# SMART-TTS/SMART-NAR_Fast_TTS

Hardware: AMD Instinct MI355X
Metric: mel_frames_per_sec (higher is better)
Workload: dtype f32

## Files before the change

smart-nar_fast_tts_amd/csrc/gemm_conv.hip:

```cpp
#include <hip/hip_ext.h>
#include <cstdlib>
#include <cstring>
#include <type_traits>
#include "rowln.h"

namespace ns {

typedef float f32x16 __attribute__((ext_vector_type(16)));
typedef unsigned u32x4g __attribute__((ext_vector_type(4)));
typedef __attribute__((address_space(3))) void* lds_ptr_t;

[[maybe_unused]] constexpr int OOR = (int)0x80000000;

template <int BM, int BN, int BK, int KS, int WGM = 2, int WGN = 2, bool ROWEPI = false, int TICKET = 0, int MF = 32>
__global__ __launch_bounds__(64 * WGM * WGN * KS) void k_conv_gemm(ConvGemm p, int ntn, int fl) {
#if defined(__HIP_DEVICE_COMPILE__)
  constexpr int NW = WGM * WGN;
  constexpr int WM = BM / WGM, WN = BN / WGN;
  constexpr int TM = WM / MF, TN = WN / MF;
  constexpr int NR = MF == 32 ? 16 : 4;
  constexpr int LG = 64 / MF;
  constexpr int KG = 4 * LG;
  constexpr int CPR = BK / 4;
  constexpr int RPI = 64 / CPR;
  static_assert(MF == 32 || MF == 16, "MFMA tile edge");
  static_assert(TM >= 1 && TN >= 1 && WM % MF == 0 && WN % MF == 0 && BM % RPI == 0 && BN % RPI == 0 && BK % KG == 0, "tile / wave-grid geometry");
  constexpr int FSH = (BK == 64) ? 0 : (BK == 32) ? 1 : 2;
  constexpr int FMSK = CPR - 1;
  static_assert(BK == 64 || BK == 32 || BK == 16, "BK");
  constexpr int EPR = 2 * BK;
  constexpr int NPASS = (BM + EPR - 1) / EPR;
  static_assert(!ROWEPI || (KS == 1 && BN % 256 == 0 && (BM % EPR) % NW == 0 && (BM < EPR || EPR % NW == 0)), "row epilogue: every pass's rows divide over the waves");
  static_assert(!(ROWEPI && TICKET), "a full-row tile needs no ticket");
  using acc_t = typename std::conditional<MF == 32, f32x16, f32x4>::type;
  constexpr bool ACC2 = TM * TN * NR <= 32;

  __shared__ __attribute__((aligned(16))) float As0[KS * BM * BK];
  __shared__ __attribute__((aligned(16))) float As1[KS * BM * BK];
  __shared__ __attribute__((aligned(16))) float Bs0[KS * BN * BK];
  __shared__ __attribute__((aligned(16))) float Bs1[KS * BN * BK];

  const int nblk = gridDim.x, bid = blockIdx.x;
  const int q8 = nblk >> 3, r8 = nblk & 7, xcd = bid & 7;
  int pos = (xcd < r8 ? xcd * (q8 + 1) : r8 * (q8 + 1) + (xcd - r8) * q8) + (bid >> 3);
  const int ntm = nblk / ntn, mq = ntm >> 3, mr = ntm & 7;
  int tile_m = 0, tile_n = 0, mstart = 0;
  for (int x = 0; x < 8; ++x) {
    const int gm = mq + (x < mr ? 1 : 0), gsz = gm * ntn;
    if (pos < gsz) {
      tile_n = pos / gm;
      tile_m = mstart + pos % gm;
      break;
    }
    pos -= gsz;
    mstart += gm;
  }
  const int m0 = tile_m * BM, n0 = tile_n * BN;

  const int tid = threadIdx.x, lane = tid & 63;
  const int wall = __builtin_amdgcn_readfirstlane(tid >> 6);
  const int grp = wall / NW, wid = wall % NW;
  const int wm0 = (wid / WGN) * WM, wn0 = (wid % WGN) * WN;

  const int Kt = p.ldw ? p.ldw : p.KW * p.Cin;
  const int cpj = p.Cin / BK;
  const int nch = p.KW * cpj;

  const __amdgpu_buffer_rsrc_t rsA = __builtin_amdgcn_make_buffer_rsrc(
      (void*)(p.X + ((ptrdiff_t)m0 - p.pad) * p.ldx), (short)0, 0x7FFFFFFF, 0x00020000);
  const __amdgpu_buffer_rsrc_t rsB =
      __builtin_amdgcn_make_buffer_rsrc((void*)(p.W + (size_t)n0 * Kt), (short)0, 0x7FFFFFFF, 0x00020000);

  constexpr int TOTA = BM / RPI, TOTB = BN / RPI;
  constexpr int IA = (TOTA + NW - 1) / NW, IB = (TOTB + NW - 1) / NW;
  constexpr bool A_EVEN = TOTA % NW == 0, B_EVEN = TOTB % NW == 0;
  const int lr = lane / CPR, ls = lane % CPR;
  auto ea = [&](int i) { return A_EVEN ? wid * IA + i : i * NW + wid; };
  auto eb = [&](int i) { return B_EVEN ? wid * IB + i : i * NW + wid; };
  int a_base[IA];
  unsigned a_jlo[IA], a_jn[IA];
#pragma unroll
  for (int i = 0; i < IA; ++i) {
    const int r = ea(i) * RPI + lr;
    const int m = m0 + r;
    int t = -1, sw = p.S;
    if (m < p.M) {
      const int mg = m + p.m_base;
      if (p.rm.row_t) { t = p.rm.row_t[mg]; sw = p.rm.row_w[mg]; }
      else t = mg % p.S;
    }
    a_base[i] = (r * p.ldx + (ls ^ ((r >> FSH) & FMSK)) * 4) * 4;
    const int jlo = max(0, p.pad - t), jhi = min(p.KW, sw + p.pad - t);
    a_jlo[i] = (unsigned)jlo;
    a_jn[i] = (t >= 0 && jhi > jlo) ? (unsigned)(jhi - jlo) : 0u;
  }
  int vb[IB];
#pragma unroll
  for (int i = 0; i < IB; ++i) {
    const int r = eb(i) * RPI + lr;
    vb[i] = (n0 + r < p.N) ? (r * Kt + (ls ^ ((r >> FSH) & FMSK)) * 4) * 4 : OOR;
  }
  auto dma_chunk = [&](float* As, float* Bs, int ch) {
    const int cc = ch / p.KW, j = ch - cc * p.KW;
    const int soA = (cc * BK + j * p.ldx) * 4, soB = (j * p.Cin + cc * BK) * 4;
#pragma unroll
    for (int i = 0; i < IA; ++i) {
      const int va = ((unsigned)j - a_jlo[i] < a_jn[i]) ? a_base[i] : OOR;
      if (A_EVEN || ea(i) < TOTA)
        __builtin_amdgcn_raw_ptr_buffer_load_lds(rsA, (lds_ptr_t)&As[ea(i) * RPI * BK], 16, va, soA, 0, 0);
    }
#pragma unroll
    for (int i = 0; i < IB; ++i) {
      if (B_EVEN || eb(i) < TOTB)
        __builtin_amdgcn_raw_ptr_buffer_load_lds(rsB, (lds_ptr_t)&Bs[eb(i) * RPI * BK], 16, vb[i], soB, 0, 0);
    }
  };

  acc_t acc[TM][TN];
#pragma unroll
  for (int mi = 0; mi < TM; ++mi)
#pragma unroll
    for (int ni = 0; ni < TN; ++ni)
#pragma unroll
      for (int r = 0; r < NR; ++r) acc[mi][ni][r] = 0.f;
  [[maybe_unused]] acc_t tot[ACC2 ? TM : 1][ACC2 ? TN : 1];
  if constexpr (ACC2) {
#pragma unroll
    for (int mi = 0; mi < TM; ++mi)
#pragma unroll
      for (int ni = 0; ni < TN; ++ni)
#pragma unroll
        for (int r = 0; r < NR; ++r) tot[mi][ni][r] = 0.f;
  }

  [[maybe_unused]] float bvp[TN];
  if constexpr (KS == 1) {
#pragma unroll
    for (int ni = 0; ni < TN; ++ni) {
      const int n = n0 + wn0 + ni * MF + (lane & (MF - 1));
      bvp[ni] = (p.bias && n < p.N) ? p.bias[n] : 0.f;
    }
  }

  const int frow = lane & (MF - 1), fh = lane / MF;
  int foff[BK / KG];
#pragma unroll
  for (int g = 0; g < BK / KG; ++g) foff[g] = frow * BK + (((LG * g + fh) ^ ((frow >> FSH) & FMSK)) * 4);

  float* const A0 = As0 + grp * BM * BK;
  float* const A1 = As1 + grp * BM * BK;
  float* const B0 = Bs0 + grp * BN * BK;
  float* const B1 = Bs1 + grp * BN * BK;

  const int nsteps = (nch + KS - 1) / KS;
  if (grp < nch) dma_chunk(A0, B0, grp);
  __syncthreads();

  auto step = [&](auto fresh_c, int st, const float* Ac, const float* Bc, float* An, float* Bn) {
    constexpr bool FRESH = decltype(fresh_c)::value;
    const acc_t zero = {};
    const int ch = st * KS + grp;
    if (ch + KS < nch) dma_chunk(An, Bn, ch + KS);
    if (KS == 1 || ch < nch) {
      const float* as = Ac + wm0 * BK;
      const float* bs = Bc + wn0 * BK;
#pragma unroll
      for (int g = 0; g < BK / KG; ++g) {
        if constexpr (MF == 32) {
          f32x4 a[TM], b[TN];
#pragma unroll
          for (int mi = 0; mi < TM; ++mi) a[mi] = *reinterpret_cast<const f32x4*>(as + mi * 32 * BK + foff[g]);
#pragma unroll
          for (int ni = 0; ni < TN; ++ni) b[ni] = *reinterpret_cast<const f32x4*>(bs + ni * 32 * BK + foff[g]);
#pragma unroll
          for (int e = 0; e < 4; ++e)
#pragma unroll
            for (int mi = 0; mi < TM; ++mi)
#pragma unroll
              for (int ni = 0; ni < TN; ++ni)
                acc[mi][ni] = __builtin_amdgcn_mfma_f32_32x32x2f32(a[mi][e], b[ni][e], (FRESH && g == 0 && e == 0) ? zero : acc[mi][ni], 0, 0, 0);
        } else {
          f32x4 b[TN];
#pragma unroll
          for (int ni = 0; ni < TN; ++ni) b[ni] = *reinterpret_cast<const f32x4*>(bs + ni * 16 * BK + foff[g]);
#pragma unroll
          for (int mi = 0; mi < TM; ++mi) {
            const f32x4 a = *reinterpret_cast<const f32x4*>(as + mi * 16 * BK + foff[g]);
#pragma unroll
            for (int e = 0; e < 4; ++e)
#pragma unroll
              for (int ni = 0; ni < TN; ++ni)
                acc[mi][ni] = __builtin_amdgcn_mfma_f32_16x16x4f32(a[e], b[ni][e], (FRESH && g == 0 && e == 0) ? zero : acc[mi][ni], 0, 0, 0);
          }
        }
      }
    } else if constexpr (FRESH) {
#pragma unroll
      for (int mi = 0; mi < TM; ++mi)
#pragma unroll
        for (int ni = 0; ni < TN; ++ni) acc[mi][ni] = zero;
    }
    __syncthreads();
  };
  int due = fl;
  bool fresh = false;
  constexpr std::false_type CONT{};
  constexpr std::true_type OPEN{};
  for (int st = 0; st < nsteps; st += 2) {
    if (ACC2 && fresh) step(OPEN, st, A0, B0, A1, B1);
    else step(CONT, st, A0, B0, A1, B1);
    if (st + 1 < nsteps) step(CONT, st + 1, A1, B1, A0, B0);
    if constexpr (ACC2) {
      due -= 2;
      fresh = due == 0 && st + 2 < nsteps;
      if (fresh) {
        due = fl;
#pragma unroll
        for (int mi = 0; mi < TM; ++mi)
#pragma unroll
          for (int ni = 0; ni < TN; ++ni) tot[mi][ni] += acc[mi][ni];
      }
    }
  }
  if constexpr (ACC2) {
#pragma unroll
    for (int mi = 0; mi < TM; ++mi)
#pragma unroll
      for (int ni = 0; ni < TN; ++ni) acc[mi][ni] = tot[mi][ni] + acc[mi][ni];
  }

  const int ecol = lane & (MF - 1);
  auto crow = [&](int r) { return MF == 32 ? (r & 3) + 8 * (r >> 2) + 4 * (lane >> 5) : r + 4 * (lane >> 4); };
  if constexpr (KS > 1) {
    constexpr int RS = BN + 8, TILE = BM * RS;
    constexpr int PB = (KS * BN * BK) / TILE, PA = (KS * BM * BK) / TILE;
    static_assert(2 * PB + 2 * PA >= KS, "the KS partial tiles must fit the four staging objects, whole tiles per object");
    auto part = [&](int g) -> float* {
      if (g < PB) return Bs0 + g * TILE;
      if (g < 2 * PB) return Bs1 + (g - PB) * TILE;
      if (g < 2 * PB + PA) return As0 + (g - 2 * PB) * TILE;
      return As1 + (g - 2 * PB - PA) * TILE;
    };
    constexpr int NT = 64 * NW * KS, U = BM * BN / 4, UPT = (U + NT - 1) / NT, CPRW = BN / 4;
    f32x4 bia[UPT], res[UPT];
#pragma unroll
    for (int k = 0; k < UPT; ++k) {
      const int u = tid + k * NT, row = u / CPRW, m = m0 + row, n = n0 + (u % CPRW) * 4;
      const bool ok = u < U && m < p.M && n < p.N;
      bia[k] = (ok && p.bias) ? *reinterpret_cast<const f32x4*>(p.bias + n) : f32x4{0.f, 0.f, 0.f, 0.f};
      res[k] = (ok && p.resid) ? *reinterpret_cast<const f32x4*>(p.resid + (size_t)m * p.ldr + n) : f32x4{0.f, 0.f, 0.f, 0.f};
    }
    {
      float* mine = part(grp);
#pragma unroll
      for (int mi = 0; mi < TM; ++mi)
#pragma unroll
        for (int ni = 0; ni < TN; ++ni)
#pragma unroll
          for (int r = 0; r < NR; ++r)
            mine[(wm0 + mi * MF + crow(r)) * RS + wn0 + ni * MF + ecol] = acc[mi][ni][r];
    }
    __syncthreads();
    [[maybe_unused]] const __amdgpu_buffer_rsrc_t rsYs = __builtin_amdgcn_make_buffer_rsrc((void*)p.Y, (short)0, 0x7FFFFFFF, 0x00020000);
#pragma unroll
    for (int k = 0; k < UPT; ++k) {
      const int u = tid + k * NT, row = u / CPRW, c4 = u % CPRW, m = m0 + row, n = n0 + c4 * 4;
      if (u >= U || m >= p.M || n >= p.N) continue;
      f32x4 v = *reinterpret_cast<const f32x4*>(part(0) + row * RS + c4 * 4);
#pragma unroll
      for (int g2 = 1; g2 < KS; ++g2) v += *reinterpret_cast<const f32x4*>(part(g2) + row * RS + c4 * 4);
      v += bia[k];
      if (p.act == ACT_RELU) {
#pragma unroll
        for (int e = 0; e < 4; ++e) v[e] = v[e] > 0.f ? v[e] : 0.f;
      } else if (p.act == ACT_TANH) {
#pragma unroll
        for (int e = 0; e < 4; ++e) v[e] = tanhf(v[e]);
      }
      if (p.resid) v += res[k];
      if constexpr (TICKET != 0) __builtin_amdgcn_raw_buffer_store_b128(__builtin_bit_cast(u32x4g, v), rsYs, (m * p.ldy + n) * 4, 0, 16 );
      else *reinterpret_cast<f32x4*>(p.Y + (size_t)m * p.ldy + n) = v;
    }
  }

  if constexpr (ROWEPI) {
    static_assert(WGM == 1, "full-row tiles put their waves side by side");
    auto trow = [&](int ml) -> float* { return (ml < BK ? Bs0 : Bs1) + (ml % BK) * BN; };
    constexpr int NV = BN / 256;
    f32x4 lng[NV], lnb[NV];
#pragma unroll
    for (int i = 0; i < NV; ++i) {
      lng[i] = *reinterpret_cast<const f32x4*>(p.e.ln_g + lane * 4 + i * 256);
      lnb[i] = *reinterpret_cast<const f32x4*>(p.e.ln_b + lane * 4 + i * 256);
    }
    const RowEpilogue& e2 = p.e;
    auto pass = [&](auto pc) {
      constexpr int P = decltype(pc)::value;
      constexpr int P0 = P * EPR, PR = (BM - P0 < EPR ? BM - P0 : EPR), RPW = PR / NW;
      if constexpr (P > 0) __syncthreads();
      const int mw = m0 + P0 + wid * RPW;
      f32x4 rv[RPW][NV];
#pragma unroll
      for (int rr = 0; rr < RPW; ++rr) {
        const int m = mw + rr;
#pragma unroll
        for (int i = 0; i < NV; ++i) {
          rv[rr][i] = f32x4{0.f, 0.f, 0.f, 0.f};
          if (p.resid && m < p.M) rv[rr][i] = *reinterpret_cast<const f32x4*>(p.resid + (size_t)m * p.ldr + lane * 4 + i * 256);
        }
      }
      int tt[RPW];
      unsigned keep[RPW];
      int mv = mw;
      asm("" : "+v"(mv));
      row_batch_masks<RPW>(p.e, p.M, p.S, mv, 1, tt, keep);
#pragma unroll
      for (int ni = 0; ni < TN; ++ni) {
        const int nl = wn0 + ni * MF + ecol;
        const float bv = bvp[ni];
#pragma unroll
        for (int mi = 0; mi < TM; ++mi) {
          if ((mi * MF) / EPR != P) continue;
#pragma unroll
          for (int r = 0; r < NR; ++r) {
            const int ml = mi * MF + crow(r) - P0;
            float v = acc[mi][ni][r] + bv;
            if (p.act == ACT_RELU) v = v > 0.f ? v : 0.f;
            else if (p.act == ACT_TANH) v = tanhf(v);
            trow(ml)[nl] = v;
          }
        }
      }
      __syncthreads();
      f32x4 v[RPW][NV];
#pragma unroll
      for (int rr = 0; rr < RPW; ++rr)
#pragma unroll
        for (int i = 0; i < NV; ++i) {
          v[rr][i] = *reinterpret_cast<const f32x4*>(trow(wid * RPW + rr) + lane * 4 + i * 256);
          if (p.resid) v[rr][i] += rv[rr][i];
        }
      row_batch_finish<NV, RPW>(v, tt, keep, lane, p.epi, e2, p.M, mv, 1, lng, lnb);
    };
    pass(std::integral_constant<int, 0>{});
    if constexpr (NPASS > 1) pass(std::integral_constant<int, 1>{});
    if constexpr (NPASS > 2) pass(std::integral_constant<int, 2>{});
    if constexpr (NPASS > 3) pass(std::integral_constant<int, 3>{});
    static_assert(NPASS <= 4, "row epilogue: at most 4 parking passes (BM <= 8 BK)");
  } else {
    if constexpr (KS == 1) {
#pragma unroll
    for (int ni = 0; ni < TN; ++ni) {
      const int n = n0 + wn0 + ni * MF + ecol;
      if (n >= p.N) continue;
      const float bv = bvp[ni];
#pragma unroll
      for (int mi = 0; mi < TM; ++mi) {
        float rs[NR];
#pragma unroll
        for (int r = 0; r < NR; ++r) {
          const int m = m0 + wm0 + mi * MF + crow(r);
          rs[r] = (p.resid && m < p.M) ? p.resid[(size_t)m * p.ldr + n] : 0.f;
        }
#pragma unroll
        for (int r = 0; r < NR; ++r) {
          const int m = m0 + wm0 + mi * MF + crow(r);
          if (m >= p.M) continue;
          float v = acc[mi][ni][r] + bv;
          if (p.act == ACT_RELU) v = v > 0.f ? v : 0.f;
          else if (p.act == ACT_TANH) v = tanhf(v);
          if (p.resid) v += rs[r];
          if constexpr (TICKET) __hip_atomic_store(p.Y + (size_t)m * p.ldy + n, v, __ATOMIC_RELAXED, __HIP_MEMORY_SCOPE_AGENT);
          else p.Y[(size_t)m * p.ldy + n] = v;
        }
      }
    }
    }
    if constexpr (TICKET) {
      constexpr int NWALL = NW * KS;
      asm volatile("s_waitcnt vmcnt(0)" ::: "memory");
      __syncthreads();
      int* const last = reinterpret_cast<int*>(As0);
      if (tid == 0) *last = __hip_atomic_fetch_add(p.e.ticket + tile_m, 1, __ATOMIC_RELAXED, __HIP_MEMORY_SCOPE_AGENT) == ntn - 1;
      __syncthreads();
      if (!*last) return;
      const __amdgpu_buffer_rsrc_t rsY = __builtin_amdgcn_make_buffer_rsrc((void*)p.Y, (short)0, p.M * p.ldy * 4, 0x00020000);
      constexpr int RPW = BM / NWALL, RB = RPW < 8 ? RPW : 8;
      static_assert(BM % NWALL == 0 && RPW % RB == 0, "rows divide evenly over the waves");
#pragma unroll
      for (int j0 = 0; j0 < RPW; j0 += RB)
        row_epilogue_batch<TICKET, RB>(rsY, p.ldy, lane, p.epi, p.e, p.M, p.S, m0 + wall + j0 * NWALL, NWALL);
    }
  }
#endif
}

int conv_gemm_acc_chunk() {
  static const int v = [] {
    const char* e = getenv("NS_ACC_CHUNK");
    int k = e ? atoi(e) : 64;
    if (k < 0 || k % 64 != 0) k = 64;
    return k;
  }();
  return v;
}
static int acc_chunk_k() { return conv_gemm_acc_chunk(); }
static int long_k_threshold() {
  static const int v = [] { const char* e = getenv("NS_LONG_K"); const int k = e ? atoi(e) : 512; return k >= 256 ? k : 256; }();
  return v;
}
static constexpr bool tile_chunks(int bm, int bn, int waves) { return bm * bn / (64 * waves) <= 32; }

struct LaunchRecord { int n; int out[2][8]; };
static thread_local LaunchRecord* t_describe = nullptr;

template <int BM, int BN, int BK, int KS = 1, int WGM = 2, int WGN = 2, bool ROWEPI = false, int TICKET = 0, int MF = 32>
static hipError_t launch_t(const ConvGemm& p, hipStream_t st, const LaunchTiming* tm = nullptr) {
  if (LaunchRecord* r = t_describe) {
    if (r->n < 2) {
      const int form[8] = {BM, BN, BK, KS, MF, ROWEPI ? 1 : 0, TICKET, p.M};
      for (int i = 0; i < 8; ++i) r->out[r->n][i] = form[i];
    }
    r->n++;
    return hipSuccess;
  }
  const int ntm = (p.M + BM - 1) / BM, ntn = (p.N + BN - 1) / BN;
  const int fl = ((acc_chunk_k() / BK) + 1) & ~1;
  if (tm && (tm->start || tm->stop))
    hipExtLaunchKernelGGL((k_conv_gemm<BM, BN, BK, KS, WGM, WGN, ROWEPI, TICKET, MF>), dim3(ntm * ntn), dim3(64 * WGM * WGN * KS), 0, st, tm->start, tm->stop, 0, p, ntn, fl);
  else
    hipLaunchKernelGGL((k_conv_gemm<BM, BN, BK, KS, WGM, WGN, ROWEPI, TICKET, MF>), dim3(ntm * ntn), dim3(64 * WGM * WGN * KS), 0, st, p, ntn, fl);
  return hipGetLastError();
}

bool conv_gemm_ticket_ok(int M, int N, int Cin) {
  return M > 0 && (N == 256 || N == 512) && Cin % 32 == 0 && (long long)M * N * 4 < (1ll << 31) && (long)((M + 31) / 32) * ((N + 127) / 128) <= 512;
}

bool conv_gemm_row_epilogue_ok(int M, int N, int Cin) {
  return M > 0 && (N == 256 || N == 512) && Cin % 32 == 0;
}

bool launch_planner_enabled() {
  static const bool on = [] { const char* e = getenv("NS_PLAN"); return !(e && e[0] == '0'); }();
  return on;
}

static ConvGemm row_range(const ConvGemm& p, int begin, int count) {
  ConvGemm q = p;
  q.X += (size_t)begin * p.ldx;
  q.Y += (size_t)begin * p.ldy;
  if (q.resid) q.resid += (size_t)begin * p.ldr;
  q.M = count;
  q.m_base = p.m_base + begin;
  return q;
}

struct TileModel { int bm, bn; float a0, a1, b0, b1; };
enum TileId { T256, T128, T64W, T64, T64N, T32, N_TILES };
static constexpr TileModel kTile[N_TILES] = {
    {256, 256, 11.0f, 0.00f, 10.0f, 7.25f},
    {128, 256, 5.0f, 0.20f, 8.0f, 3.60f},
    {64, 256, 6.0f, 0.17f, 3.6f, 1.83f},
    {64, 128, 5.5f, 0.09f, 1.6f, 0.93f},
    {64, 64, 5.0f, 0.20f, 1.2f, 0.46f},
    {32, 128, 5.0f, 0.23f, 1.0f, 0.45f},
};
static long tile_wgs(int t, long M, int N) { return ((M + kTile[t].bm - 1) / kTile[t].bm) * ((N + kTile[t].bn - 1) / kTile[t].bn); }
static float tile_time(int t, long M, int N, int chunks) {
  const long steps = (tile_wgs(t, M, N) + 255) / 256;
  const float a = kTile[t].a0 + kTile[t].a1 * chunks, b = kTile[t].b0 + kTile[t].b1 * chunks;
  const float more = (t == T64N || t == T32) ? 1.15f : 1.0f;
  return (a + b + b * more * (float)(steps - 1)) * (1.0f + 0.01f * (float)t);
}
enum TileFam { F32 = 0, F16W = 1, F16N = 2 };
struct TileSel { int fam, id; };
static int sel_bm(TileSel t) { return t.fam == F32 ? kTile[t.id].bm : 16 * t.id; }
static int sel_bn(TileSel t) { return t.fam == F32 ? kTile[t.id].bn : t.fam == F16W ? 256 : 128; }
constexpr int F16W_MIN = 3, F16W_MAX = 16, F16N_MIN = 3, F16N_MAX = 10;
static bool tile16_enabled() {
  static const bool on = [] { const char* e = getenv("NS_TILE16"); return !(e && e[0] == '0'); }();
  return on;
}
bool conv_gemm_tile16_enabled() { return launch_planner_enabled() && tile16_enabled(); }
static bool tile16n_enabled() {
  static const bool on = [] { const char* e = getenv("NS_TILE16N"); return !(e && e[0] == '0'); }();
  return on;
}
static float tile16_time(int fam, int slabs, long M, int N, int chunks) {
  const int bm = 16 * slabs, bn = fam == F16W ? 256 : 128;
  const long wgs = ((M + bm - 1) / bm) * ((N + bn - 1) / bn);
  const float steps = (float)((wgs + 255) / 256);
  const float rows = (float)bm * (fam == F16W ? 1.0f : 0.5f);
  const float b1 = 0.0281f * rows * (fam == F16N ? 1.02f : 1.0f);
  return 5.0f + 0.0016f * rows * (float)chunks + steps * (8.0f + b1 * (float)chunks);
}
template <int S>
static hipError_t launch_f16w(const ConvGemm& p, hipStream_t st, const LaunchTiming* tm) { return launch_t<16 * S, 256, 32, 1, 1, 16, false, 0, 16>(p, st, tm); }
template <int S>
static hipError_t launch_f16n(const ConvGemm& p, hipStream_t st, const LaunchTiming* tm) { return launch_t<16 * S, 128, 32, 1, 1, 8, false, 0, 16>(p, st, tm); }
static hipError_t launch_tile(TileSel t, const ConvGemm& p, hipStream_t st, const LaunchTiming* tm) {
  if (t.fam == F16W) {
    switch (t.id) {
      case 3: return launch_f16w<3>(p, st, tm); case 4: return launch_f16w<4>(p, st, tm); case 5: return launch_f16w<5>(p, st, tm);
      case 6: return launch_f16w<6>(p, st, tm); case 7: return launch_f16w<7>(p, st, tm); case 8: return launch_f16w<8>(p, st, tm);
      case 9: return launch_f16w<9>(p, st, tm); case 10: return launch_f16w<10>(p, st, tm); case 11: return launch_f16w<11>(p, st, tm);
      case 12: return launch_f16w<12>(p, st, tm); case 13: return launch_f16w<13>(p, st, tm); case 14: return launch_f16w<14>(p, st, tm);
      case 15: return launch_f16w<15>(p, st, tm); case 16: return launch_f16w<16>(p, st, tm);
      default: return hipErrorInvalidValue;
    }
  }
  if (t.fam == F16N) {
    switch (t.id) {
      case 3: return launch_f16n<3>(p, st, tm); case 4: return launch_f16n<4>(p, st, tm); case 5: return launch_f16n<5>(p, st, tm);
      case 6: return launch_f16n<6>(p, st, tm); case 7: return launch_f16n<7>(p, st, tm); case 8: return launch_f16n<8>(p, st, tm);
      case 9: return launch_f16n<9>(p, st, tm); case 10: return launch_f16n<10>(p, st, tm);
      default: return hipErrorInvalidValue;
    }
  }
  switch (t.id) {
    case T256: return launch_t<256, 256, 32, 1, 8, 2>(p, st, tm);
    case T128: return launch_t<128, 256, 32, 1, 4, 4>(p, st, tm);
    case T64W: return launch_t<64, 256, 32, 1, 2, 4>(p, st, tm);
    case T64: return launch_t<64, 128, 32, 1, 2, 4>(p, st, tm);
    case T64N: return launch_t<64, 64, 32, 1, 2, 2>(p, st, tm);
    default: return launch_t<32, 128, 32, 1, 1, 4>(p, st, tm);
  }
}
struct RowPlan { TileSel main; int main_rows; TileSel rem; float us; };
static RowPlan plan_rows(long M, int N, int chunks) {
  constexpr float CUT_US = 3.0f;
  RowPlan best{{F32, -1}, 0, {F32, T64}, 1e30f};
  const bool long_k = chunks * 32 > long_k_threshold() && acc_chunk_k() > 0;
  const int first = chunks <= 16 ? T64W : long_k ? T128 : T256;
  for (int t = first; t < N_TILES; ++t) {
    if (kTile[t].bn > N && t != T32 && t != T64N && t != T64) continue;
    const float c = tile_time(t, M, N, chunks);
    if (c < best.us) best = RowPlan{{F32, -1}, 0, {F32, t}, c};
  }
  for (int t = first; t <= T64; ++t) {
    if (kTile[t].bn > N) continue;
    const long ntn = (N + kTile[t].bn - 1) / kTile[t].bn;
    const long per = (256 / ntn) * kTile[t].bm;
    if (per <= 0) continue;
    for (long k = M / per; k >= 1 && k >= M / per - 1; --k) {
      const long rows = k * per, rest = M - rows;
      if (rest <= 0) continue;
      const float cm = tile_time(t, rows, N, chunks);
      for (int r = t + 1; r < N_TILES; ++r) {
        if (kTile[r].bn > N && r < T64) continue;
        const float c = cm + CUT_US + tile_time(r, rest, N, chunks);
        if (c < best.us) best = RowPlan{{F32, t}, (int)rows, {F32, r}, c};
      }
    }
  }
  if (tile16_enabled()) {
    float margin = 1.01f;
    if (best.main_rows == 0 && best.rem.fam == F32) {
      const long w = tile_wgs(best.rem.id, M, N);
      if ((double)w / (double)(((w + 255) / 256) * 256) >= 0.9) margin = 1.03f;
    }
    const int w_max = long_k ? 8 : F16W_MAX, n_max = long_k ? 8 : F16N_MAX;
    if (N % 256 == 0)
      for (int sl = F16W_MIN; sl <= w_max; ++sl) {
        const float c = tile16_time(F16W, sl, M, N, chunks) * margin;
        if (c < best.us) best = RowPlan{{F32, -1}, 0, {F16W, sl}, c};
      }
    if (N % 128 == 0 && tile16n_enabled())
      for (int sl = F16N_MIN; sl <= n_max; ++sl) {
        const float c = tile16_time(F16N, sl, M, N, chunks) * margin;
        if (c < best.us) best = RowPlan{{F32, -1}, 0, {F16N, sl}, c};
      }
  }
  return best;
}

bool conv_gemm_plan(int M, int N, int Cin, int KW, int out[8]) {
  if (!launch_planner_enabled() || M <= 0 || N < 128 || Cin % 32 != 0) return false;
  const long rows64 = ((long)M + 63) / 64;
  if (rows64 * ((N + 127) / 128) <= 256) return false;
  const RowPlan pl = plan_rows(M, N, KW * (Cin / 32));
  const TileSel mt = pl.main_rows ? pl.main : pl.rem;
  out[0] = sel_bm(mt); out[1] = sel_bn(mt); out[2] = pl.main_rows ? pl.main_rows : M;
  out[3] = pl.main_rows ? sel_bm(pl.rem) : 0; out[4] = pl.main_rows ? sel_bn(pl.rem) : 0; out[5] = pl.main_rows ? M - pl.main_rows : 0;
  out[6] = mt.fam == F32 ? 32 : 16;
  out[7] = (int)(pl.us + 0.5f);
  return true;
}

int conv_gemm_row_tile(int M, int N, int K) {
  if (!launch_planner_enabled() || !tile16_enabled()) return 32;
  const int top = N > 256 ? 48 : 112;
  (void)K;
  long best = 32 * ((((long)M + 31) / 32 + 255) / 256);
  int bm = 32;
  for (int c = 48; c <= top; c += 32) {
    const long rows = (long)c * ((((long)M + c - 1) / c + 255) / 256);
    if (rows < best) { best = rows; bm = c; }
  }
  return bm;
}

static hipError_t launch_conv_gemm_impl(const ConvGemm& p_in, hipStream_t st, bool allow_split, const LaunchTiming* tm);
static hipError_t launch_tall(const ConvGemm& p, hipStream_t st, const LaunchTiming* tm) {
  if (p.KW * p.Cin > 256 && acc_chunk_k() > 0) return launch_t<128, 256, 32, 1, 4, 4>(p, st, tm);
  return launch_t<256, 256, 32, 1, 8, 2>(p, st, tm);
}
hipError_t launch_conv_gemm(const ConvGemm& p, hipStream_t st, const LaunchTiming* tm) { return launch_conv_gemm_impl(p, st, true, tm); }

static hipError_t launch_conv_gemm_impl(const ConvGemm& p_in, hipStream_t st, bool allow_split, const LaunchTiming* tm) {
  ConvGemm p = p_in;
  if (p.M <= 0 || p.N <= 0) return hipSuccess;
  if (p.m_base != 0 && p.epi != EPI_NONE) return hipErrorInvalidValue;
  if (p.ldw == 0) p.ldw = p.KW * p.Cin;
  if (p.Cin % 16 != 0 || (p.ldx & 3) != 0 || (p.ldw & 3) != 0 || p.ldw < p.KW * p.Cin) return hipErrorInvalidValue;
  if ((p.N & 3) != 0 || (p.ldy & 3) != 0 || (p.resid && (p.ldr & 3) != 0)) return hipErrorInvalidValue;
  if ((long long)(256 + p.KW) * p.ldx >= (1ll << 29) || (long long)512 * p.ldw >= (1ll << 29)) return hipErrorInvalidValue;
  if (p.epi != EPI_NONE && p.e.ticket) {
    if (!conv_gemm_ticket_ok(p.M, p.N, p.Cin) || p.ldy != p.N || (p.resid && (p.ldr & 3)) || (p.epi == EPI_LN && !p.e.y_out)) return hipErrorInvalidValue;
    const long rows32 = (p.M + 31) / 32;
    auto wgs = [&](long rows, int bn) { return rows * ((p.N + bn - 1) / bn); };
    const int nch = p.KW * (p.Cin / 32);
#define NS_TICKET_LADDER(NVT)                                                                                                        \
    if (wgs(rows32, 32) <= 256) return nch >= 16 ? launch_t<32, 32, 32, 8, 1, 1, false, NVT>(p, st, tm) : launch_t<32, 32, 32, 4, 1, 1, false, NVT>(p, st, tm); \
    if (wgs(rows32, 64) <= 256) return launch_t<32, 64, 32, 4, 1, 2, false, NVT>(p, st, tm);                                             \
                     \
    if (launch_planner_enabled() && tile16_enabled() && wgs((p.M + 47) / 48, 64) <= 256)                                                 \
      return launch_t<48, 64, 32, 4, 1, 2, false, NVT, 16>(p, st, tm);                                                                   \
    if (wgs(rows32, 128) <= 512) return launch_t<32, 128, 32, 2, 1, 4, false, NVT>(p, st, tm);                                           \
    return hipErrorInvalidValue;
    if (p.N == 256) { NS_TICKET_LADDER(1) }
    NS_TICKET_LADDER(2)
#undef NS_TICKET_LADDER
  }
  if (p.epi != EPI_NONE) {
    if (!conv_gemm_row_epilogue_ok(p.M, p.N, p.Cin) || (p.epi == EPI_LN && p.ldy != p.N) || (p.resid && (p.ldr & 3))) return hipErrorInvalidValue;
    p.e.y_out = p.Y;
    const int bm = conv_gemm_row_tile(p.M, p.N, p.KW * p.Cin);
    if (p.N == 256) {
      switch (bm) {
        case 48: return launch_t<48, 256, 32, 1, 1, 16, true, 0, 16>(p, st, tm);
        case 80: return launch_t<80, 256, 32, 1, 1, 16, true, 0, 16>(p, st, tm);
        case 112: return launch_t<112, 256, 32, 1, 1, 16, true, 0, 16>(p, st, tm);
        default: return launch_t<32, 256, 32, 1, 1, 8, true>(p, st, tm);
      }
    }
    if (bm == 48) return launch_t<48, 512, 32, 1, 1, 16, true, 0, 16>(p, st, tm);
    return launch_t<32, 512, 32, 1, 1, 16, true>(p, st, tm);
  }
  const bool bk32 = (p.Cin % 32) == 0;
  const long rows64 = (p.M + 63) / 64, rows32 = (p.M + 31) / 32;
  auto wgs = [&](long rows, int bn) { return rows * ((p.N + bn - 1) / bn); };
  if (bk32 && p.N > 64 && p.N <= 96 && p.KW * p.Cin >= 1024) {
    if (launch_planner_enabled()) {
      if (wgs(rows32, 64) > 256) {
        if (tile16_enabled() && rows32 > 256 && (p.M + 47) / 48 <= 256) return launch_t<48, 96, 32, 4, 1, 3, false, 0, 16>(p, st, tm);
        if (tile16_enabled() && rows32 > 512 && (p.M + 79) / 80 <= 256) return launch_t<80, 96, 32, 1, 5, 3, false, 0, 16>(p, st, tm);
        return launch_t<32, 96, 32, 4, 1, 3>(p, st, tm);
      }
    } else {
      if (rows64 >= 512) return launch_t<64, 96, 32, 1, 2, 3>(p, st, tm);
      if (rows32 >= 400) return launch_t<32, 96, 32, 4, 1, 3>(p, st, tm);
    }
  }
  if (launch_planner_enabled() && allow_split && bk32 && p.N >= 128 && wgs(rows64, 128) > 256) {
    const RowPlan pl = plan_rows(p.M, p.N, p.KW * (p.Cin / 32));
    if (pl.main_rows == 0) return launch_tile(pl.rem, p, st, tm);
    const LaunchTiming t0{tm ? tm->start : nullptr, nullptr}, t1{nullptr, tm ? tm->stop : nullptr};
    const hipError_t e = launch_tile(pl.main, row_range(p, 0, pl.main_rows), st, &t0);
    if (e != hipSuccess) return e;
    return launch_tile(pl.rem, row_range(p, pl.main_rows, p.M - pl.main_rows), st, &t1);
  }
  if (bk32 && p.N >= 512 && p.KW * p.Cin <= 512 && wgs(rows64, 128) > 256) return launch_t<64, 128, 32, 1, 2, 4>(p, st, tm);
  if (bk32 && p.N >= 512 && wgs(rows64, 256) >= 400) {
    auto fill = [](long n) { return (double)n / (double)(((n + 255) / 256) * 256); };
    const long c256 = wgs((p.M + 255) / 256, 256), c128 = wgs((p.M + 127) / 128, 256);
    if (c256 >= 200 && c256 <= 512 && fill(c256) >= 0.95) return launch_tall(p, st, tm);
    if (c128 <= 512 && fill(c128) >= 0.95) return launch_t<128, 256, 32, 1, 4, 4>(p, st, tm);
    const long ntn = (p.N + 255) / 256, per = 256 / ntn;
    if (allow_split && p.epi == EPI_NONE && per >= 1 && p.M > 256 * per && wgs(rows64, 256) < 4 * 512) {
      const long r256 = 256 * per;
      const long n = p.M / r256 > 2 ? 2 : p.M / r256;
      const LaunchTiming t0{tm ? tm->start : nullptr, nullptr}, t1{nullptr, tm ? tm->stop : nullptr};
      const hipError_t e = launch_tall(row_range(p, 0, (int)(n * r256)), st, &t0);
      if (e != hipSuccess) return e;
      return launch_conv_gemm_impl(row_range(p, (int)(n * r256), (int)(p.M - n * r256)), st, false, &t1);
    }
  }
  if (bk32 && p.N >= 512 && wgs(rows64, 256) >= 400) {
    const long sc = (wgs(rows64, 256) + 255) / 256, sd = (wgs(rows64, 128) + 255) / 256;
    if (sc <= 8 && p.N % 128 == 0 && (double)sd * 0.5 < 0.93 * (double)sc) return launch_t<64, 128, 32, 1, 2, 4>(p, st, tm);
    return launch_t<64, 256, 32, 1, 2, 4>(p, st, tm);
  }
  if (bk32 && p.N >= 128 && wgs(rows64, 128) > 256) return launch_t<64, 128, 32, 1, 2, 4>(p, st, tm);
  if (!allow_split && bk32 && p.N >= 128) return launch_t<64, 128, 32, 1, 2, 4>(p, st, tm);
  if (bk32) {
    const int nch = p.KW * (p.Cin / 32);
    if (wgs(rows32, 32) <= 256) return nch >= 16 ? launch_t<32, 32, 32, 8, 1, 1>(p, st, tm) : launch_t<32, 32, 32, 4, 1, 1>(p, st, tm);
    if (wgs(rows32, 64) <= 256) return launch_t<32, 64, 32, 4, 1, 2>(p, st, tm);
    const bool row_width = p.N == 256 || p.N == 512;
    if (row_width && launch_planner_enabled() && tile16_enabled() && wgs((p.M + 47) / 48, 64) <= 256)
      return launch_t<48, 64, 32, 4, 1, 2, false, 0, 16>(p, st, tm);
    if (wgs(rows32, 128) <= 512) {
      if (!row_width && launch_planner_enabled() && tile16_enabled() && wgs(rows32, 128) > 256 && wgs((p.M + 47) / 48, 128) <= 256)
        return launch_t<48, 128, 32, 2, 1, 4, false, 0, 16>(p, st, tm);
      return launch_t<32, 128, 32, 2, 1, 4>(p, st, tm);
    }
    return launch_t<64, 64, 32>(p, st, tm);
  }
  if (wgs(rows32, 32) <= 512) return launch_t<32, 32, 16, 4, 1, 1>(p, st, tm);
  if (p.N >= 256 && wgs(rows64, 256) >= 1024) return launch_t<64, 256, 16, 1, 2, 4>(p, st, tm);
  if (p.N >= 128 && wgs(rows64, 128) >= 512) return launch_t<64, 128, 16, 1, 2, 4>(p, st, tm);
  return launch_t<64, 64, 16>(p, st, tm);
}

int conv_gemm_describe(int M, int N, int Cin, int KW, int epi, int out[2][8]) {
  static int ticket_tag;
  static float y_out_tag;
  for (int l = 0; l < 2; ++l)
    for (int i = 0; i < 8; ++i) out[l][i] = 0;
  if (M <= 0 || N <= 0 || Cin <= 0 || KW <= 0 || epi < 0 || epi > 2) return 0;
  ConvGemm p;
  memset(&p, 0, sizeof(p));
  p.ldx = Cin; p.ldy = N; p.M = M; p.N = N; p.Cin = Cin; p.KW = KW; p.pad = (KW - 1) / 2; p.S = M;
  p.epi = epi ? EPI_LN : EPI_NONE;
  if (epi == 2) { p.e.ticket = &ticket_tag; p.e.y_out = &y_out_tag; }
  LaunchRecord rec;
  memset(&rec, 0, sizeof(rec));
  t_describe = &rec;
  const hipError_t e = launch_conv_gemm_impl(p, nullptr, true, nullptr);
  t_describe = nullptr;
  if (e != hipSuccess || rec.n > 2) return 0;
  for (int l = 0; l < rec.n; ++l)
    for (int i = 0; i < 8; ++i) out[l][i] = rec.out[l][i];
  return rec.n;
}

}
```

Before: 2.945 million.

## Issue first weight DMA before row-map lookups and hoist row-epilogue operand loads

For split-K and row-epilogue conv GEMM variants, the first B-tile DMA is now issued before the A-row index lookups finish, so the weight fetch overlaps the dependent row_t/row_w gathers. The row-epilogue operands (LayerNorm gamma/beta, residual rows, mask batches) are now loaded before the last K pair, or right after the K loop, when a register budget check allows it. This hides their global-load latency behind MFMA work. The cost is higher register pressure and more complex control flow in the prologue and main loop.

```diff
diff --git a/smart-nar_fast_tts_amd/csrc/gemm_conv.hip b/smart-nar_fast_tts_amd/csrc/gemm_conv.hip
--- a/smart-nar_fast_tts_amd/csrc/gemm_conv.hip
+++ b/smart-nar_fast_tts_amd/csrc/gemm_conv.hip
@@ -77,22 +77,33 @@
   const int lr = lane / CPR, ls = lane % CPR;
   auto ea = [&](int i) { return A_EVEN ? wid * IA + i : i * NW + wid; };
   auto eb = [&](int i) { return B_EVEN ? wid * IB + i : i * NW + wid; };
+  constexpr bool EARLY = ROWEPI || KS > 1;
   int a_base[IA];
   unsigned a_jlo[IA], a_jn[IA];
-#pragma unroll
-  for (int i = 0; i < IA; ++i) {
-    const int r = ea(i) * RPI + lr;
-    const int m = m0 + r;
+  int a_t[IA], a_sw[IA];
+  auto a_lookup = [&](int i) __attribute__((always_inline)) {
+    const int m = m0 + ea(i) * RPI + lr;
     int t = -1, sw = p.S;
     if (m < p.M) {
       const int mg = m + p.m_base;
       if (p.rm.row_t) { t = p.rm.row_t[mg]; sw = p.rm.row_w[mg]; }
       else t = mg % p.S;
     }
+    a_t[i] = t;
+    a_sw[i] = sw;
+  };
+  auto a_entry = [&](int i) __attribute__((always_inline)) {
+    const int r = ea(i) * RPI + lr;
+    const int t = a_t[i], sw = a_sw[i];
     a_base[i] = (r * p.ldx + (ls ^ ((r >> FSH) & FMSK)) * 4) * 4;
     const int jlo = max(0, p.pad - t), jhi = min(p.KW, sw + p.pad - t);
     a_jlo[i] = (unsigned)jlo;
     a_jn[i] = (t >= 0 && jhi > jlo) ? (unsigned)(jhi - jlo) : 0u;
+  };
+#pragma unroll
+  for (int i = 0; i < IA; ++i) {
+    a_lookup(i);
+    if constexpr (!EARLY) a_entry(i);
   }
   int vb[IB];
 #pragma unroll
@@ -100,63 +111,78 @@
     const int r = eb(i) * RPI + lr;
     vb[i] = (n0 + r < p.N) ? (r * Kt + (ls ^ ((r >> FSH) & FMSK)) * 4) * 4 : OOR;
   }
-  auto dma_chunk = [&](float* As, float* Bs, int ch) {
+  auto dma_a = [&](float* As, int ch) __attribute__((always_inline)) {
     const int cc = ch / p.KW, j = ch - cc * p.KW;
-    const int soA = (cc * BK + j * p.ldx) * 4, soB = (j * p.Cin + cc * BK) * 4;
+    const int soA = (cc * BK + j * p.ldx) * 4;
 #pragma unroll
     for (int i = 0; i < IA; ++i) {
       const int va = ((unsigned)j - a_jlo[i] < a_jn[i]) ? a_base[i] : OOR;
       if (A_EVEN || ea(i) < TOTA)
         __builtin_amdgcn_raw_ptr_buffer_load_lds(rsA, (lds_ptr_t)&As[ea(i) * RPI * BK], 16, va, soA, 0, 0);
     }
+  };
+  auto dma_b = [&](float* Bs, int ch) __attribute__((always_inline)) {
+    const int cc = ch / p.KW, j = ch - cc * p.KW;
+    const int soB = (j * p.Cin + cc * BK) * 4;
 #pragma unroll
     for (int i = 0; i < IB; ++i) {
       if (B_EVEN || eb(i) < TOTB)
         __builtin_amdgcn_raw_ptr_buffer_load_lds(rsB, (lds_ptr_t)&Bs[eb(i) * RPI * BK], 16, vb[i], soB, 0, 0);
     }
   };
-
-  acc_t acc[TM][TN];
-#pragma unroll
-  for (int mi = 0; mi < TM; ++mi)
-#pragma unroll
-    for (int ni = 0; ni < TN; ++ni)
-#pragma unroll
-      for (int r = 0; r < NR; ++r) acc[mi][ni][r] = 0.f;
-  [[maybe_unused]] acc_t tot[ACC2 ? TM : 1][ACC2 ? TN : 1];
-  if constexpr (ACC2) {
-#pragma unroll
-    for (int mi = 0; mi < TM; ++mi)
-#pragma unroll
-      for (int ni = 0; ni < TN; ++ni)
-#pragma unroll
-        for (int r = 0; r < NR; ++r) tot[mi][ni][r] = 0.f;
-  }
-
-  [[maybe_unused]] float bvp[TN];
-  if constexpr (KS == 1) {
-#pragma unroll
-    for (int ni = 0; ni < TN; ++ni) {
-      const int n = n0 + wn0 + ni * MF + (lane & (MF - 1));
-      bvp[ni] = (p.bias && n < p.N) ? p.bias[n] : 0.f;
-    }
-  }
-
-  const int frow = lane & (MF - 1), fh = lane / MF;
-  int foff[BK / KG];
-#pragma unroll
-  for (int g = 0; g < BK / KG; ++g) foff[g] = frow * BK + (((LG * g + fh) ^ ((frow >> FSH) & FMSK)) * 4);
-
+  auto dma_chunk = [&](float* As, float* Bs, int ch) __attribute__((always_inline)) {
+    dma_a(As, ch);
+    dma_b(Bs, ch);
+  };
   float* const A0 = As0 + grp * BM * BK;
   float* const A1 = As1 + grp * BM * BK;
   float* const B0 = Bs0 + grp * BN * BK;
   float* const B1 = Bs1 + grp * BN * BK;
+  if constexpr (EARLY) {
+    if (grp < nch) dma_b(B0, grp);
+#pragma unroll
+    for (int i = 0; i < IA; ++i) a_entry(i);
+    if (grp < nch) dma_a(A0, grp);
+  }
+
+  acc_t acc[TM][TN];
+#pragma unroll
+  for (int mi = 0; mi < TM; ++mi)
+#pragma unroll
+    for (int ni = 0; ni < TN; ++ni)
+#pragma unroll
+      for (int r = 0; r < NR; ++r) acc[mi][ni][r] = 0.f;
+  [[maybe_unused]] acc_t tot[ACC2 ? TM : 1][ACC2 ? TN : 1];
+  if constexpr (ACC2) {
+#pragma unroll
+    for (int mi = 0; mi < TM; ++mi)
+#pragma unroll
+      for (int ni = 0; ni < TN; ++ni)
+#pragma unroll
+        for (int r = 0; r < NR; ++r) tot[mi][ni][r] = 0.f;
+  }
+
+  [[maybe_unused]] float bvp[TN];
+  if constexpr (KS == 1) {
+#pragma unroll
+    for (int ni = 0; ni < TN; ++ni) {
+      const int n = n0 + wn0 + ni * MF + (lane & (MF - 1));
+      bvp[ni] = (p.bias && n < p.N) ? p.bias[n] : 0.f;
+    }
+  }
+
+  const int frow = lane & (MF - 1), fh = lane / MF;
+  int foff[BK / KG];
+#pragma unroll
+  for (int g = 0; g < BK / KG; ++g) foff[g] = frow * BK + (((LG * g + fh) ^ ((frow >> FSH) & FMSK)) * 4);
 
   const int nsteps = (nch + KS - 1) / KS;
-  if (grp < nch) dma_chunk(A0, B0, grp);
+  if constexpr (!EARLY) {
+    if (grp < nch) dma_chunk(A0, B0, grp);
+  }
   __syncthreads();
 
-  auto step = [&](auto fresh_c, int st, const float* Ac, const float* Bc, float* An, float* Bn) {
+  auto step = [&](auto fresh_c, int st, const float* Ac, const float* Bc, float* An, float* Bn) __attribute__((always_inline)) {
     constexpr bool FRESH = decltype(fresh_c)::value;
     const acc_t zero = {};
     const int ch = st * KS + grp;
@@ -206,7 +232,7 @@
   bool fresh = false;
   constexpr std::false_type CONT{};
   constexpr std::true_type OPEN{};
-  for (int st = 0; st < nsteps; st += 2) {
+  auto pair = [&](int st) __attribute__((always_inline)) {
     if (ACC2 && fresh) step(OPEN, st, A0, B0, A1, B1);
     else step(CONT, st, A0, B0, A1, B1);
     if (st + 1 < nsteps) step(CONT, st + 1, A1, B1, A0, B0);
@@ -221,6 +247,44 @@
           for (int ni = 0; ni < TN; ++ni) tot[mi][ni] += acc[mi][ni];
       }
     }
+  };
+  constexpr int NV = ROWEPI ? BN / 256 : 1;
+  constexpr int RPW0 = ROWEPI ? (BM < EPR ? BM : EPR) / NW : 1;
+  [[maybe_unused]] f32x4 lng[NV], lnb[NV], rv0[RPW0][NV];
+  [[maybe_unused]] int tt0[RPW0], mv0 = 0;
+  [[maybe_unused]] unsigned keep0[RPW0];
+  [[maybe_unused]] auto row_operands = [&](int mw, auto& rv, auto& tt, auto& keep, int& mv) __attribute__((always_inline)) {
+    constexpr int R = std::extent<typename std::remove_reference<decltype(tt)>::type>::value;
+#pragma unroll
+    for (int rr = 0; rr < R; ++rr) {
+      const int m = mw + rr;
+#pragma unroll
+      for (int i = 0; i < NV; ++i) {
+        rv[rr][i] = f32x4{0.f, 0.f, 0.f, 0.f};
+        if (p.resid && m < p.M) rv[rr][i] = *reinterpret_cast<const f32x4*>(p.resid + (size_t)m * p.ldr + lane * 4 + i * 256);
+      }
+    }
+    mv = mw;
+    asm("" : "+v"(mv));
+    row_batch_masks<R>(p.e, p.M, p.S, mv, 1, tt, keep);
+  };
+  constexpr bool HOIST = ROWEPI && (ACC2 ? 2 : 1) * TM * TN * NR + 4 * (RPW0 + 2) * NV <= 64;
+  [[maybe_unused]] auto epilogue_operands = [&]() __attribute__((always_inline)) {
+#pragma unroll
+    for (int i = 0; i < NV; ++i) {
+      lng[i] = *reinterpret_cast<const f32x4*>(p.e.ln_g + lane * 4 + i * 256);
+      lnb[i] = *reinterpret_cast<const f32x4*>(p.e.ln_b + lane * 4 + i * 256);
+    }
+    row_operands(m0 + wid * RPW0, rv0, tt0, keep0, mv0);
+  };
+  if constexpr (HOIST) {
+    int st = 0;
+    for (; st + 2 < nsteps; st += 2) pair(st);
+    epilogue_operands();
+    if (st < nsteps) pair(st);
+  } else {
+    for (int st = 0; st < nsteps; st += 2) pair(st);
+    if constexpr (ROWEPI) epilogue_operands();
   }
   if constexpr (ACC2) {
 #pragma unroll
@@ -286,34 +350,10 @@
   if constexpr (ROWEPI) {
     static_assert(WGM == 1, "full-row tiles put their waves side by side");
     auto trow = [&](int ml) -> float* { return (ml < BK ? Bs0 : Bs1) + (ml % BK) * BN; };
-    constexpr int NV = BN / 256;
-    f32x4 lng[NV], lnb[NV];
-#pragma unroll
-    for (int i = 0; i < NV; ++i) {
-      lng[i] = *reinterpret_cast<const f32x4*>(p.e.ln_g + lane * 4 + i * 256);
-      lnb[i] = *reinterpret_cast<const f32x4*>(p.e.ln_b + lane * 4 + i * 256);
-    }
     const RowEpilogue& e2 = p.e;
-    auto pass = [&](auto pc) {
+    auto rows = [&](auto pc, auto& rv, auto& tt, auto& keep, int mv) __attribute__((always_inline)) {
       constexpr int P = decltype(pc)::value;
       constexpr int P0 = P * EPR, PR = (BM - P0 < EPR ? BM - P0 : EPR), RPW = PR / NW;
-      if constexpr (P > 0) __syncthreads();
-      const int mw = m0 + P0 + wid * RPW;
-      f32x4 rv[RPW][NV];
-#pragma unroll
-      for (int rr = 0; rr < RPW; ++rr) {
-        const int m = mw + rr;
-#pragma unroll
-        for (int i = 0; i < NV; ++i) {
-          rv[rr][i] = f32x4{0.f, 0.f, 0.f, 0.f};
-          if (p.resid && m < p.M) rv[rr][i] = *reinterpret_cast<const f32x4*>(p.resid + (size_t)m * p.ldr + lane * 4 + i * 256);
-        }
-      }
-      int tt[RPW];
-      unsigned keep[RPW];
-      int mv = mw;
-      asm("" : "+v"(mv));
-      row_batch_masks<RPW>(p.e, p.M, p.S, mv, 1, tt, keep);
 #pragma unroll
       for (int ni = 0; ni < TN; ++ni) {
         const int nl = wn0 + ni * MF + ecol;
@@ -341,6 +381,20 @@
           if (p.resid) v[rr][i] += rv[rr][i];
         }
       row_batch_finish<NV, RPW>(v, tt, keep, lane, p.epi, e2, p.M, mv, 1, lng, lnb);
+    };
+    auto pass = [&](auto pc) __attribute__((always_inline)) {
+      constexpr int P = decltype(pc)::value;
+      if constexpr (P == 0) {
+        rows(pc, rv0, tt0, keep0, mv0);
+      } else {
+        constexpr int P0 = P * EPR, PR = (BM - P0 < EPR ? BM - P0 : EPR), RPW = PR / NW;
+        __syncthreads();
+        f32x4 rv[RPW][NV];
+        int tt[RPW], mv;
+        unsigned keep[RPW];
+        row_operands(m0 + P0 + wid * RPW, rv, tt, keep, mv);
+        rows(pc, rv, tt, keep, mv);
+      }
     };
     pass(std::integral_constant<int, 0>{});
     if constexpr (NPASS > 1) pass(std::integral_constant<int, 1>{});
```

Result: no change. 2.945 million, median of 2 (+0.0%).
